# pingcap-incubator/tinysql

Hardware: AMD Instinct MI355X
Metric: probed rows/sec on int64-key inner hash join (higher is better)
Workload: dtype int64; 1 GPU; SELECT count(*) FROM probe JOIN build ON k: 1e+08 x 1e+08 int64-key inner hash join per GPU, J-uniq-shuffled, hit ratio 1.0, build side resident in HBM; build key range 27 bits <= 28: packed route (2-byte entries against direct-address images) — keys beyond 28 bits (31 if unique) take the 64-bit route, see general_keys_64bit_route; probe_rows_per_gpu=100000000, build_rows_per_gpu=100000000, parallelism=single GPU

## Files before the change

### __graft_entry__.py

```python
import os
import subprocess
import sys

ROOT = os.path.dirname(os.path.abspath(__file__))
if ROOT not in sys.path:
    sys.path.insert(0, ROOT)


PIPELINED = {"tsq_join.resusage": (("k_lds_probe_count", "k_da_partition2p"), 3), "tsq_unionscan.resusage": (("k_us_",), 9),
             "tsq_lookup.resusage": (("k_lk_", "k_rg_"), 6),
             "tsq_insert.resusage": (("k_ins_", "k_aid_"), 7),
             "tsq_dupcheck.resusage": (("k_dc_", "k_rows_equal"), 17),
             "tsq_mvcc.resusage": (("k_mv_",), 12),
             "tsq_mvcc_write.resusage": (("k_mw_",), 8)}


def check_no_spills():
    import re

    total = 0
    for fname, (kernels, at_least) in PIPELINED.items():
        text = open(os.path.join(ROOT, "tinysql_amd", "csrc", fname)).read()
        seen = 0
        for m in re.finditer(r"Function Name: (\S+).*?ScratchSize \[bytes/lane\]: (\d+)", text, re.S):
            if any(k in m.group(1) for k in kernels):
                seen += 1
                if int(m.group(2)) != 0:
                    raise RuntimeError("%s spills %s bytes/lane: these kernels must not use scratch" % (m.group(1), m.group(2)))
        if seen < at_least:
            raise RuntimeError("resource-usage remarks of the kernels of %s not found (%d)" % (fname, seen))
        total += seen
    return total


def check_partition_fit():
    import re

    text = open(os.path.join(ROOT, "tinysql_amd", "csrc", "tsq_join.resusage")).read()
    seen = 0
    for m in re.finditer(r"Function Name: (\S*k_da_partition2pILi(\d+)E\S*).*?VGPRs: (\d+).*?LDS Size \[bytes/block\]: (\d+)", text, re.S):
        name, nt, vgprs, lds = m.group(1), int(m.group(2)), int(m.group(3)), int(m.group(4))
        seen += 1
        if vgprs > 128:
            raise RuntimeError("%s uses %d VGPRs: more than 128 leave fewer than 4 waves per SIMD" % (name, vgprs))
        if lds * (2 if nt == 512 else 1) > 160 * 1024:
            raise RuntimeError("%s uses %d bytes of LDS per workgroup: %d workgroup(s) per CU do not fit 160 KB" % (name, lds, 2 if nt == 512 else 1))
    if seen < 3:
        raise RuntimeError("resource-usage remarks of k_da_partition2p not found (%d)" % seen)
    return seen


def build():
    env = dict(os.environ)
    env.setdefault("HIPCC", "/opt/rocm/bin/hipcc")
    subprocess.run(["make", "-C", os.path.join(ROOT, "tinysql_amd", "csrc"), "-j4", "ARCH=gfx950"], check=True, env=env)
    check_no_spills()
    check_partition_fit()
    subprocess.run(["make", "-C", os.path.join(ROOT, "tinysql_amd", "host")], check=True)
    subprocess.run(["make", "-C", os.path.join(ROOT, "oracle")], check=True)
    subprocess.run(["make", "-C", os.path.join(ROOT, "tests", "hostsim")], check=True)
    import tinysql_amd
    from tinysql_amd import _lib
    _lib.load()


def smoke():
    import numpy as np

    from oracle import binding as orc
    from tests import gpu_helpers as G
    from tests import helpers as H
    from tinysql_amd import _abi as abi
    from tinysql_amd import _lib
    from tinysql_amd import expression as E
    from tinysql_amd.chunk import Chunk, Column

    rng = np.random.default_rng(1)
    n = 20000
    t = [abi.I64, abi.I64]
    left = Chunk([Column(abi.I64, rng.integers(0, 3000, n), rng.random(n) > 0.05), Column(abi.I64, rng.integers(-99, 99, n))])
    right = Chunk([Column(abi.I64, rng.integers(0, 3000, n), rng.random(n) > 0.05), Column(abi.I64, rng.integers(-99, 99, n))])
    with _lib.Context(0) as ctx:
        keep = []
        conds = [E.ScalarFunction("gt", E.ScalarFunction("plus", E.Column(1, abi.I64), E.Column(3, abi.I64)), E.Constant(0))]
        cfg = H.join_cfg(t, t, [0], [0], abi.JOIN_LEFT_OUTER, 1, conds, (), keep)
        want = orc.hash_join(cfg, right, left)
        got = G.run_join(ctx, cfg, right, left)
        assert H.rows_equal_unordered(got, want), "smoke: join rows differ from the oracle"
        c, s, x = G.run_join(ctx, cfg, right, left, count_only=True, checksum=True)
        assert c == want.NumRows() and (s, x) == orc.rows_checksum(want), "smoke: join checksum differs"
        aggs = [(abi.AGG_FIRSTROW, 0, abi.I64), (abi.AGG_SUM, 1, abi.I64), (abi.AGG_COUNT, -1, abi.I64)]
        acfg = H.agg_cfg(t, [0], aggs)
        assert H.rows_equal_unordered(G.run_agg(ctx, acfg, left, [abi.I64] * 3), orc.hash_agg(acfg, left, 4, 4)), "smoke: agg differs"
        from tinysql_amd.chunk import StrColumn
        words = [None if i % 7 == 0 else ("k%03d" % (i % 40)).encode() * (1 + i % 3) for i in range(n)]
        schk = Chunk([StrColumn(words), left.columns[1]])
        se = E.ScalarFunction("and", E.ScalarFunction("le", E.ScalarFunction("ifnull", E.Column(0, abi.BYTES), E.Constant("k020")), E.Constant("k020k020")),
                              E.ScalarFunction("gt", E.ScalarFunction("plus", E.ScalarFunction("length", E.Column(0, abi.BYTES)), E.Column(1, abi.I64)), E.Constant(0)))
        ce = E.CompiledExpr(ctx, [se])
        try:
            assert ce.VecEval(schk).values() == orc.expr_eval(E.compile_expr(se), schk)[0].values(), "smoke: string expression differs"
        finally:
            ce.close()
        from tinysql_amd import distsql
        raw = orc.encode_rows(left)
        dec, used = distsql.decode_rows(ctx, raw, left.types(), n)
        assert used == raw.size and dec.rows() == orc.decode_rows(raw, left.types(), n)[1].rows(), "smoke: row decode differs"
        assert G.run_sort(ctx, left, [0, 1], [False, True]).rows() == orc.sort_rows(left, [0, 1], [False, True]).rows(), "smoke: sort differs"
        from tinysql_amd import rowcodec as RC
        vals, offs = orc.rowcodec_encode(left, [1, 2])
        scan = RC.NewChunkDecoder(ctx, [RC.ColInfo(2, RC.TypeLonglong), RC.ColInfo(1, RC.TypeLonglong)]).DecodeToChunk(vals, offs)
        assert scan.rows() == orc.rowcodec_decode(vals, offs, None, [(2, abi.I64), (1, abi.I64)])[1].rows(), "smoke: stored-row decode differs"
        from tinysql_amd import tablecodec
        hs = rng.integers(-(1 << 62), 1 << 62, 1000)
        keys = tablecodec.EncodeRowKeysWithHandles(ctx, 41, hs)
        assert bytes(keys[:19]) == orc.encode_row_key(41, int(hs[0])) and (tablecodec.DecodeRowKeys(ctx, keys) == hs).all(), "smoke: record keys differ"
        resp_chunk = Chunk([left.columns[0], StrColumn(words), left.columns[1]])
        raw2, offs2 = distsql.encode_rows(ctx, resp_chunk)
        assert bytes(raw2) == bytes(orc.encode_rows(resp_chunk)), "smoke: response bytes with a string column differ"
        back = distsql.decode_chunks(ctx, distsql.response_chunks(raw2, offs2), resp_chunk.types())
        assert back.rows() == resp_chunk.rows(), "smoke: chunked response decode differs"
        from tinysql_amd import chunk_codec, coprocessor
        from tinysql_amd.gpu_pipeline import drain_device
        wire = chunk_codec.Codec(ctx, resp_chunk.types()).Encode(resp_chunk)
        assert wire == orc.WireChunk.from_chunk(resp_chunk).encode(), "smoke: wire chunk bytes differ"
        assert chunk_codec.Codec(ctx, resp_chunk.types()).Decode(wire)[0].to_chunk().rows() == resp_chunk.rows(), "smoke: wire chunk decode differs"
        ikeys, ioffs = orc.encode_index_keys(resp_chunk, 41, 2, hs[:resp_chunk.NumRows()], np.ones(resp_chunk.NumRows(), np.uint8))
        itypes = resp_chunk.types() + [abi.I64]
        iscan = coprocessor.indexScanExec(ctx, itypes, 3, coprocessor.indexScanExec.PrimaryKeyIsSigned, ikeys, ioffs)
        got_rows = [r for ch in drain_device(iscan) for r in ch.rows()]
        assert got_rows == orc.decode_index_kv(ikeys.tobytes(), ioffs, None, None, 3, itypes, 1)[1].rows(), "smoke: index scan differs"
        wchunk = Chunk([left.columns[0], StrColumn(words), left.columns[1]])
        wvals, woffs = tablecodec.EncodeRow(ctx, wchunk, [1, 2, 300])
        ovals, ooffs = orc.rowcodec_encode(wchunk, [1, 2, 300])
        assert bytes(wvals) == bytes(ovals) and (woffs == ooffs).all(), "smoke: stored-row encode differs"
        whs = np.arange(n, dtype=np.int64) - 7
        gk, gko, gv, gvo, gd = tablecodec.GenIndexKeys(ctx, 41, 3, True, Chunk(wchunk.columns[:2]), whs)
        in_key = np.array([None in r for r in Chunk(wchunk.columns[:2]).rows()])
        ok, oko = orc.encode_index_keys(Chunk(wchunk.columns[:2]), 41, 3, whs, in_key.astype(np.uint8))
        assert bytes(gk) == bytes(ok) and (gko == oko).all() and (gd == ~in_key).all() and gvo[-1] == 8 * int((~in_key).sum()) + int(in_key.sum()), "smoke: index entries differ"
        kb = Chunk([left.columns[0], StrColumn([None if i % 13 == 0 else b"w%d" % (i % 50) for i in range(n)]), left.columns[1]])
        kp = Chunk([right.columns[0], StrColumn([None if i % 11 == 0 else b"w%d" % (i % 60) for i in range(n)]), right.columns[1]])
        kcfg = H.join_cfg(kp.types(), kb.types(), [0, 1], [0, 1], abi.JOIN_LEFT_OUTER, 1)
        kstats = []
        kgot = G.run_join(ctx, kcfg, kb, kp, chunk_rows=1 << 20, radix=abi.RADIX_FORCE, stats_out=kstats)
        assert kstats[0].probe_route == abi.ROUTE_KEYREC and H.rows_equal_unordered(kgot, orc.hash_join(kcfg, kb, kp)), "smoke: key-record join differs"
        kconds = [E.ScalarFunction("gt", E.ScalarFunction("plus", E.Column(2, abi.I64), E.Column(5, abi.I64)), E.Constant(0))]
        ccfg = H.join_cfg(kp.types(), kb.types(), [0, 1], [0, 1], abi.JOIN_LEFT_OUTER, 1, kconds, (), keep)
        cstats = []
        cgot = G.run_join(ctx, ccfg, kb, kp, chunk_rows=1 << 20, radix=abi.RADIX_FORCE, stats_out=cstats)
        assert cstats[0].probe_route == abi.ROUTE_KEYREC and H.rows_equal_unordered(cgot, orc.hash_join(ccfg, kb, kp)), "smoke: key-record join with a condition differs"
        saggs = [(abi.AGG_FIRSTROW, 1, abi.BYTES), (abi.AGG_SUM, 2, abi.I64), (abi.AGG_COUNT, -1, abi.I64)]
        scfg = H.agg_cfg(kb.types(), [1], saggs)
        sstats = []
        sgot = G.run_agg(ctx, scfg, kb, [abi.BYTES, abi.I64, abi.I64], chunk_rows=1 << 20, fast=abi.AGGFAST_FORCE, stats_out=sstats)
        assert sstats[0].build_partitioned == 3 and H.rows_equal_unordered(sgot, orc.hash_agg(scfg, kb, 4, 4)), "smoke: dictionary aggregate differs"
        ordered = orc.sort_rows(left, [0], [False])
        st_got = G.run_agg(ctx, acfg, ordered, [abi.I64] * 3, stream=True)
        assert H.rows_equal_unordered(st_got, orc.hash_agg(acfg, left, 4, 4)), "smoke: stream aggregate differs"
        from tinysql_amd import executor as X
        from tinysql_amd.gpu_pipeline import DeviceChunk, DeviceTableScan, GpuUnionScanExec
        uh = np.arange(2000, dtype=np.int64) * 2
        ua = uh[::5] + 1
        dirty = X.DirtyTable()
        for h_ in ua:
            dirty.AddRow(h_)
        for h_ in uh[::7]:
            dirty.DeleteRow(h_)
        table = DeviceChunk.from_host(ctx, Chunk([Column(abi.I64, uh), Column(abi.I64, uh * 3)]))
        try:
            us = GpuUnionScanExec(ctx, DeviceTableScan(ctx, table, 512), dirty, Chunk([Column(abi.I64, ua), Column(abi.I64, ua * 3)]), [], 0, False)
            us_rows = [r for ch in drain_device(us) for r in ch.rows()]
        finally:
            table.free()
        us_want = np.sort(np.concatenate([np.setdiff1d(uh, uh[::7]), ua]))
        assert us_rows == [(int(v), int(v) * 3) for v in us_want], "smoke: union scan differs"
        from tinysql_amd.gpu_pipeline import GpuIndexLookUpExecutor
        lh = np.sort(rng.choice(np.arange(-9000, 9000), 3000, replace=False)).astype(np.int64)
        lv, lw = rng.integers(0, 500, 3000), rng.integers(-99, 99, 3000)
        lvals, loffs = tablecodec.EncodeRow(ctx, Chunk([Column(abi.I64, lv), Column(abi.I64, lw)]), [1, 2])
        ltable = coprocessor.DeviceTable(ctx, tablecodec.EncodeRowKeysWithHandles(ctx, 41, lh), lvals, loffs)
        try:
            ih = np.concatenate([lh, 20000 + np.arange(200)])
            iv = np.concatenate([lv, rng.integers(0, 500, 200)])
            io = np.lexsort((ih, iv))
            ik, iko, ivl, ivo, _ = tablecodec.GenIndexKeys(ctx, 41, 5, False, Chunk([Column(abi.I64, iv[io])]), ih[io])
            linfo = [RC.ColInfo(1, RC.TypeLonglong), RC.ColInfo(2, RC.TypeLonglong), RC.ColInfo(-1, RC.TypeLonglong, IsPKHandle=True)]
            for keep_order in (True, False):
                iscan2 = coprocessor.indexScanExec(ctx, [abi.I64, abi.I64], 1, coprocessor.indexScanExec.PrimaryKeyIsSigned, ik, iko, ivl, ivo)
                lk = GpuIndexLookUpExecutor(ctx, iscan2, ltable, linfo, [], keep_order, 64, 1024)
                lrows = [r for ch in drain_device(lk) for r in ch.rows()]
                lwant = []
                at, batch = 0, 64
                while at < ih.size:
                    th = ih[io][at:at + batch]
                    th = th[np.isin(th, lh)]
                    lwant += (th if keep_order else np.sort(th)).tolist()
                    at, batch = at + batch, min(2 * batch, 1024)
                pos = np.searchsorted(lh, np.array(lwant, dtype=np.int64))
                assert lrows == [(int(lv[p]), int(lw[p]), int(lh[p])) for p in pos], "smoke: index lookup differs (keep_order=%s)" % keep_order
        finally:
# ... 73 lines not shown
```

### tinysql_amd/csrc/tsq_join.hip

```cpp
#include "tsq_stage.h"
#include "tsq_jointable.h"
#include "tsq_buildpart.h"
#include "tsq_ldsprobe.h"
#include "tsq_keyrec.h"
#include "tsq_dajoin.h"
#include "tsq_damat.h"
#include "tsq_damat_dup.h"

#include <chrono>
#include <deque>
#include <memory>

struct KeySpec {
    int32_t n_keys;
    int32_t bidx[TSQ_MAX_KEYS];
    int32_t pidx[TSQ_MAX_KEYS];
    int32_t skip_high;
};

template <bool MULTI>
__device__ __forceinline__ bool load_kw(const tsq_colset& cs, const int32_t* idx, int n_keys, bool skip_high,
                                        int64_t row, uint64_t& kw) {
    if (!MULTI) {
        const int c = idx[0];
// ... 912 lines not shown
                    if (r->pending) { TSQ_TRY(settle_batch(j, r.get())); break; }
        } else {
            TSQ_HIP(&j->hdr, hipStreamSynchronize(ctx->stream));
            rb->copy_on = nullptr;
            rb->free_device();
            rb->on_host = true;
        }
    } else {
        TSQ_HIP(&j->hdr, hipStreamSynchronize(ctx->stream));
        for (auto& b : rb->notnull) b.release();
    }
    j->total_out += out_rows;
    j->st.out_rows += out_rows;
    j->results.push_back(std::move(rb));
    return TSQ_OK;
}

bool radix_eligible(const tsq_join* j, int64_t nrows, const uint8_t* selected_dev) {
    if (j->radix_mode == TSQ_RADIX_OFF) return false;
    if (!j->count_only || j->checksum || j->multi || j->general_cfg || j->never_match || j->chained) return false;
    if (nrows <= 0 || nrows > 0x7fffffffLL) return false;
    if (j->radix_mode == TSQ_RADIX_FORCE) return true;
    return j->nbuckets * 64 >= ((uint64_t)12 << 20) && nrows >= (4 << 20);
}

bool da_multi_ok(const tsq_join* j);
bool da_multi_count_eligible(const tsq_join* j, int64_t nrows, const uint8_t* selected_dev) {
    if (j->radix_mode == TSQ_RADIX_OFF || j->packing_mode == TSQ_RADIX_OFF || !j->multi || !da_multi_ok(j) || j->da_state < 0) return false;
    if (!j->count_only || j->checksum || j->general_cfg || j->never_match || j->chained) return false;
    if (nrows <= 0 || nrows > 0x7fffffffLL) return false;
    if (j->radix_mode == TSQ_RADIX_FORCE || j->packing_mode == TSQ_RADIX_FORCE) return true;
    return nrows >= (4 << 20);
}

struct RadixPlan {
    bool lds;
    uint32_t bits, S, nf;
};
RadixPlan radix_plan_for(const tsq_join* j) {
    RadixPlan pl{false, TSQ_RADIX_MIN_BITS, 1, 1};
    const int64_t nf_env = tsq_knob(j->ctx, TSQ_KNOB_LDS_NF_MAX, 0), pb_env = tsq_knob(j->ctx, TSQ_KNOB_RADIX_PB_MAX, 0);
    const bool want_lds = tsq_knob(j->ctx, TSQ_KNOB_RADIX_KERNEL_L2, 0) == 0;
    if (want_lds && j->tb >= TSQ_RADIX_MIN_BITS && (uint64_t)j->bs * 64 <= TSQ_LDS_IMAGE_MAX) {
        uint32_t nf_max = (uint32_t)(TSQ_LDS_IMAGE_MAX / ((uint64_t)j->bs * 64));
        if (nf_env >= 1 && (uint32_t)nf_env < nf_max) nf_max = (uint32_t)nf_env;
        uint32_t k = 0;
        while ((2u << k) <= nf_max) k++;
        int pb = (int)j->tb - (int)k;
        if (pb < TSQ_RADIX_MIN_BITS) pb = TSQ_RADIX_MIN_BITS;
        if (pb > TSQ_RADIX_MAX_BITS) pb = TSQ_RADIX_MAX_BITS;
        if (pb_env >= TSQ_RADIX_MIN_BITS && pb_env < pb) pb = (int)pb_env;
        const uint32_t fpp = 1u << (j->tb - (uint32_t)pb);
        pl.lds = true;
        pl.bits = (uint32_t)pb;
        pl.nf = fpp < nf_max ? fpp : nf_max;
        pl.S = (fpp + pl.nf - 1) / pl.nf;
        return pl;
    }
    const double slice_target = 1.5 * 1024 * 1024;
    const double parts = (double)j->nbuckets * 64.0 / slice_target;
    uint32_t bits = TSQ_RADIX_MIN_BITS;
    while (bits < 10 && (double)(1u << bits) < parts) bits++;
    if (j->tb && bits > j->tb) bits = j->tb;
    pl.bits = bits;
    return pl;
}

tsq_status batch_begin(tsq_join* j, DevEvent*& re, bool ev2 = false) {
    re = nullptr;
    if (ev2) TSQ_HIP(&j->hdr, hipEventRecord(j->ev[2], j->ctx->stream));
    const int64_t every = tsq_knob(j->ctx, TSQ_KNOB_JOIN_BATCH_TIMING, 4), b = j->st.radix_batches;
    if (every <= 0 || b % every != every - 1) return TSQ_OK;
    DevEvent* slot = j->rev[b % tsq_join::RING];
    for (int e = 0; e < 3; e++)
        TSQ_HIP(&j->hdr, slot[e].create());
    j->rev_batch1[b % tsq_join::RING] = b + 1;
    TSQ_HIP(&j->hdr, hipEventRecord(slot[0], j->ctx->stream));
    re = slot;
    return TSQ_OK;
}
tsq_status batch_mark(tsq_join* j, DevEvent* re, int e) {
    if (re) TSQ_HIP(&j->hdr, hipEventRecord(re[e], j->ctx->stream));
    return TSQ_OK;
}
tsq_status batch_end(tsq_join* j, DevEvent* re) {
    if (!re) return TSQ_OK;
    TSQ_HIP(&j->hdr, hipEventRecord(re[2], j->ctx->stream));
    j->probe_ev_slot = (int)(re - j->rev[0]) / 3;
    j->have_probe_ev = true;
    return TSQ_OK;
}
tsq_status radix_probe(tsq_join* j, const tsq_colset& pcs, int64_t nrows) {
    tsq_ctx* ctx = j->ctx;
    tsq_handle_hdr* h = &j->hdr;
    RadixStore st;
    memset(&st, 0, sizeof st);
    const RadixPlan pl = radix_plan_for(j);
    st.bits = pl.bits;
    st.R = 8;
    const uint32_t P = 1u << st.bits;
    constexpr int NT = 1024, K = 16, T = NT * K;
    const double lam = (double)nrows / ((double)P * 8.0);
    st.cap = (uint32_t)(lam * 1.08 + 8.0 * sqrt(lam) + 2.0 * T / 64.0 + 64.0);
    st.cap = (st.cap + 15u) & ~15u;
    const size_t nregions = (size_t)P * 8;
    if (nregions * st.cap >= 0xffffffffULL) return tsq_fail(h, TSQ_ERR_UNSUPPORTED, "radix probe batch too large");
    const size_t ctl_words32 = nregions + 16;
    const size_t ctl_bytes = ((ctl_words32 * 4 + 511) & ~(size_t)511) + 8 * TSQ_RADIX_QSTRIDE * 8;
    TSQ_TRY(j->rkeys.reserve(ctx, h, nregions * st.cap * 8 + 256));
    TSQ_TRY(j->rctl.reserve(ctx, h, ctl_bytes));
    TSQ_TRY(j->rvend.reserve(ctx, h, nregions * 4));
    TSQ_TRY(j->rovf.reserve(ctx, h, (size_t)nrows * 8 + 64));
    st.keys = j->rkeys.as<uint64_t>();
    st.cursor = j->rctl.as<uint32_t>();
    st.ovf_count = st.cursor + nregions;
    st.queue = (unsigned long long*)((char*)j->rctl.p + ((ctl_words32 * 4 + 511) & ~(size_t)511));
    st.valid_end = j->rvend.as<uint32_t>();
    st.ovf_keys = j->rovf.as<uint64_t>();
    st.ovf_cap = (uint32_t)nrows;
    j->da_ctl_dirty();
    TSQ_HIP(h, hipMemsetAsync(j->rctl.p, 0, ctl_bytes, ctx->stream));
    TSQ_HIP(h, hipMemsetAsync(j->rvend.p, 0xff, nregions * 4, ctx->stream));

    RadixSrc src;
    memset(&src, 0, sizeof src);
    const int kc = j->ks.pidx[0];
    src.data = pcs.data[kc];
    src.nulls = pcs.nulls[kc];
    src.type = pcs.type[kc];
    src.skip_high = j->ks.skip_high;
    src.nrows = nrows;
    const int64_t ntiles = (nrows + T - 1) / T;
    const int pgrid = (int)std::min<int64_t>(ntiles, ctx->num_cus);
    DevEvent* re;
    TSQ_TRY(batch_begin(j, re));
    hipLaunchKernelGGL((k_radix_partition<NT, K, 4, 0, false, true>), dim3(pgrid), dim3(NT), 0, ctx->stream, src, st);
    TSQ_HIP(h, hipGetLastError());
    TSQ_TRY(batch_mark(j, re, 1));
    RadixProbeArgs pa;
    memset(&pa, 0, sizeof pa);
    pa.st = st;
    fill_table(j, pa.t);
    pa.counters = j->counters.as<unsigned long long>();
    if (pl.lds) {
        constexpr int LNT = 1024;
        LdsProbeArgs la;
        memset(&la, 0, sizeof la);
        la.st = st;
        la.t = pa.t;
        la.S = pl.S;
        la.nf = pl.nf;
        la.unique = j->unique ? 1u : 0u;
        la.counters = pa.counters;
        const size_t lds = (size_t)pl.nf * j->bs * 64 + (size_t)(LNT / 64) * TSQ_LDS_RING_BYTES;
        const int lgrid = std::max(1, ctx->num_cus / 8) * 8;
        if (tsq_knob(ctx, TSQ_KNOB_LDS_PROF, 0) != 0) {
            DevBuf pb;
            TSQ_TRY(pb.reserve(ctx, h, 64));
            la.prof = pb.as<unsigned long long>();
            TSQ_HIP(h, hipMemsetAsync(pb.p, 0, 64, ctx->stream));
            TSQ_HIP(h, hipFuncSetAttribute((const void*)k_lds_probe_count<LNT, true>, hipFuncAttributeMaxDynamicSharedMemorySize, (int)lds));
            hipLaunchKernelGGL((k_lds_probe_count<LNT, true>), dim3(lgrid), dim3(LNT), lds, ctx->stream, la);
            unsigned long long pf[8];
            TSQ_HIP(h, hipMemcpyAsync(ctx->pinned + 24, pb.p, 64, hipMemcpyDeviceToHost, ctx->stream));
            TSQ_HIP(h, hipStreamSynchronize(ctx->stream));
            memcpy(pf, ctx->pinned + 24, 64);
            pb.release();
            const double nw = (double)lgrid * (LNT / 64);
            fprintf(stderr, "[lds-prof] P=2^%u S=%u nf=%u bs=%u waves=%.0f | per wave kcycles: imageA %.1f loadwait %.1f step %.1f probe %.1f drainB %.1f total %.1f | probes/wave %.0f\n",
                    st.bits, pl.S, pl.nf, j->bs, nw, pf[0] / nw / 1e3, pf[1] / nw / 1e3, pf[2] / nw / 1e3, pf[3] / nw / 1e3, pf[4] / nw / 1e3, pf[5] / nw / 1e3, pf[6] / nw);
        } else {
            TSQ_HIP(h, hipFuncSetAttribute((const void*)k_lds_probe_count<LNT>, hipFuncAttributeMaxDynamicSharedMemorySize, (int)lds));
            hipLaunchKernelGGL((k_lds_probe_count<LNT>), dim3(lgrid), dim3(LNT), lds, ctx->stream, la);
        }
    } else {
        const int per_xcd = std::max(1, ctx->num_cus / 8) * 6;
        hipLaunchKernelGGL((k_radix_probe_count<2>), dim3(per_xcd * 8), dim3(256), 0, ctx->stream, pa);
    }
    TSQ_HIP(h, hipGetLastError());
    hipLaunchKernelGGL(k_radix_probe_ovf, dim3(ctx->num_cus), dim3(256), 0, ctx->stream, pa);
    TSQ_HIP(h, hipGetLastError());
    TSQ_TRY(batch_end(j, re));
    j->st.kernel_launches += 3;
    j->st.radix_batches++;
    j->st.radix_bits = (int32_t)st.bits;
    j->st.probe_route = pl.lds ? TSQ_ROUTE_RADIX_LDS : TSQ_ROUTE_RADIX_L2;
    return TSQ_OK;
}

struct DaGeom {
    uint32_t P, cap;
    size_t nregions, ent_bytes, ctl_bytes;
};
DaGeom da_geometry(uint32_t pbits, uint32_t ebits, int64_t nrows, int T) {
    DaGeom g;
    g.P = 1u << pbits;
    const double tiles = ceil((double)nrows / T);
    const double lam = std::max((double)nrows / ((double)g.P * 8.0), ceil(tiles / 8.0) * std::min<double>((double)T, (double)nrows) / (double)g.P);
    g.cap = (uint32_t)(lam * 1.08 + 8.0 * sqrt(lam) + 2.0 * T / 64.0 + 64.0);
    g.cap = (g.cap + 63u) & ~63u;
    g.nregions = (size_t)g.P * 8;
    g.ent_bytes = g.nregions * g.cap * (ebits > 16 ? 4 : 2) + 256;
    g.ctl_bytes = ((g.nregions + 16) * 4 + 511) & ~(size_t)511;
    return g;
}

template <class... P, class... A>
hipError_t da_launch(void (*fn)(P...), dim3 grid, dim3 block, size_t lds, hipStream_t stream, const A&... args) {
    if (lds) {
        const hipError_t e = hipFuncSetAttribute((const void*)fn, hipFuncAttributeMaxDynamicSharedMemorySize, (int)lds);
        if (e != hipSuccess) return e;
    }
    hipLaunchKernelGGL(fn, grid, block, lds, stream, args...);
    return hipGetLastError();
}
struct DaBuildTimer {
    tsq_join* j;
    DevEvent e0, e1;
    explicit DaBuildTimer(tsq_join* j_) : j(j_) {}
    hipError_t start() {
        hipError_t e = e0.create();
        if (e == hipSuccess) e = e1.create();
        return e == hipSuccess ? hipEventRecord(e0, j->ctx->stream) : e;
    }
    hipError_t stop() { return hipEventRecord(e1, j->ctx->stream); }
    ~DaBuildTimer() {
        float ms = 0;
        if (e0 && e1 && hipEventElapsedTime(&ms, e0, e1) == hipSuccess) j->da_build_ms += ms;
    }
};
DaStore da_store(const tsq_join* j, const DaGeom& g, int64_t rows, void* ent, void* ctl, void* vend, void* ovf) {
    DaStore st;
    memset(&st, 0, sizeof st);
    st.ent = ent;
    st.cursor = (uint32_t*)ctl;
    st.ovf_count = st.cursor + g.nregions;
    st.valid_end = (uint32_t*)vend;
    st.ovf = (uint32_t*)ovf;
    st.ovf_cap = (uint32_t)rows;
    st.bits = j->da_pbits;
    st.ebits = j->da_ebits;
    st.cap = g.cap;
    return st;
}
hipError_t da_clear(tsq_ctx* ctx, void* ctl, void* vend, const DaGeom& g) {
    const hipError_t e = hipMemsetAsync(ctl, 0, g.ctl_bytes, ctx->stream);
    return e == hipSuccess ? hipMemsetAsync(vend, 0xff, g.nregions * 4, ctx->stream) : e;
}
struct DaBuildStore {
    DevBuf ent, idx, ctl, vend, ovf, ovfi, nnm, pay[TSQ_DA_MAXCOLS];
    tsq_status reserve(tsq_join* j, const DaGeom& g, int64_t nb, bool ids, int ncols = -1, bool nulls = false) {
        tsq_ctx* ctx = j->ctx;
        tsq_handle_hdr* h = &j->hdr;
        const size_t slots = g.nregions * g.cap;
        tsq_status s = ent.reserve(ctx, h, g.ent_bytes);
        if (s == TSQ_OK && ids) s = idx.reserve(ctx, h, slots * 4 + 256);
        if (s == TSQ_OK) s = ctl.reserve(ctx, h, g.ctl_bytes);
        if (s == TSQ_OK) s = vend.reserve(ctx, h, g.nregions * 4);
        if (s == TSQ_OK) s = ovf.reserve(ctx, h, (size_t)nb * 4 + 64);
        if (s == TSQ_OK && (ids || ncols >= 0)) s = ovfi.reserve(ctx, h, (size_t)nb * 4 + 64);
        for (int v = 0; v < ncols && s == TSQ_OK; v++) s = pay[v].reserve(ctx, h, slots * 8 + 256);
        if (s == TSQ_OK && nulls) s = nnm.reserve(ctx, h, slots + 256);
        return s;
    }
    DaStore store(const tsq_join* j, const DaGeom& g, int64_t nb) const {
        DaStore st = da_store(j, g, nb, ent.p, ctl.p, vend.p, ovf.p);
        st.idx = idx.as<uint32_t>();
        st.ovf_idx = ovfi.as<uint32_t>();
        return st;
    }
    DaColStore col_store(const tsq_join* j, const DaGeom& g, int64_t nb, int ncols, bool nulls) const {
        DaColStore cs;
        memset(&cs, 0, sizeof cs);
        cs.st = store(j, g, nb);
        cs.st.miss_count = cs.st.ovf_count + 1;
        for (int v = 0; v < ncols; v++) cs.pay[v] = pay[v].as<uint64_t>();
        cs.nnmask = nulls ? nnm.as<uint8_t>() : nullptr;
        return cs;
    }
    hipError_t clear(tsq_ctx* ctx, const DaGeom& g) { return da_clear(ctx, ctl.p, vend.p, g); }
};
enum DaIds { DA_IDS_NONE, DA_IDS_LISTS, DA_IDS_ALL };
tsq_status da_probe_store(tsq_join* j, const DaGeom& g, int64_t nrows, DaIds ids, bool miss, DaStore& st) {
    tsq_ctx* ctx = j->ctx;
    tsq_handle_hdr* h = &j->hdr;
    TSQ_TRY(j->rkeys.reserve(ctx, h, g.ent_bytes));
    if (ids == DA_IDS_ALL) TSQ_TRY(j->ridx.reserve(ctx, h, g.nregions * g.cap * 4 + 256));
    TSQ_TRY(j->rctl.reserve(ctx, h, g.ctl_bytes));
    TSQ_TRY(j->rvend.reserve(ctx, h, g.nregions * 4));
    TSQ_TRY(j->rovf.reserve(ctx, h, (size_t)nrows * 4 + 64));
    if (ids != DA_IDS_NONE) TSQ_TRY(j->rovfidx.reserve(ctx, h, (size_t)nrows * 4 + 64));
    if (miss) TSQ_TRY(j->rmiss.reserve(ctx, h, (size_t)nrows * 4 + 64));
    st = da_store(j, g, nrows, j->rkeys.p, j->rctl.p, j->rvend.p, j->rovf.p);
    if (ids == DA_IDS_ALL) st.idx = j->ridx.as<uint32_t>();
    if (ids != DA_IDS_NONE) {
        st.ovf_idx = j->rovfidx.as<uint32_t>();
        st.miss_count = st.ovf_count + 1;
        st.miss = j->rmiss.as<uint32_t>();
    }
    return TSQ_OK;
}
tsq_status da_clear_batch(tsq_join* j, const DaGeom& g) {
    tsq_ctx* ctx = j->ctx;
    tsq_handle_hdr* h = &j->hdr;
    const size_t n_pc = (size_t)g.P + 1;
    TSQ_TRY(j->tkcnt.reserve(ctx, h, n_pc * 8 + 64));
    j->da_ctl_dirty();
    TSQ_HIP(h, da_clear(ctx, j->rctl.p, j->rvend.p, g));
    TSQ_HIP(h, hipMemsetAsync(j->tkcnt.p, 0, n_pc * 8, ctx->stream));
    TSQ_HIP(h, hipMemsetAsync(ctx->dscratch + 52, 0, 16, ctx->stream));
    return TSQ_OK;
}
struct DaSizes {
    int64_t part_rows, ovf_rows, miss_rows;
};
tsq_status da_queue_sizes(tsq_join* j, const DaStore& st, const unsigned long long* total, const void* ovf, size_t ovf_bytes) {
    tsq_ctx* ctx = j->ctx;
    tsq_handle_hdr* h = &j->hdr;
    ctx->pinned[53] = 0;
    TSQ_HIP(h, hipMemcpyAsync(ctx->pinned + 52, total, 8, hipMemcpyDeviceToHost, ctx->stream));
    TSQ_HIP(h, hipMemcpyAsync(ctx->pinned + 53, ovf, ovf_bytes, hipMemcpyDeviceToHost, ctx->stream));
    TSQ_HIP(h, hipMemcpyAsync(ctx->pinned + 54, st.miss_count, 4, hipMemcpyDeviceToHost, ctx->stream));
    return TSQ_OK;
}
tsq_status da_wait_sizes(tsq_join* j, bool outer, DaSizes& z) {
    tsq_ctx* ctx = j->ctx;
// ... 3532 lines not shown
```

### tinysql_amd/csrc/tsq_ldsprobe.h

```cpp
#ifndef TSQ_LDSPROBE_H
#define TSQ_LDSPROBE_H

#include "tsq_radix.h"

#define TSQ_LDS_IMAGE_MAX (128 * 1024)
#define TSQ_LDS_RING 128
#define TSQ_LDS_RING_BYTES (TSQ_LDS_RING * 10)
#define TSQ_LDS_RING_BYTES_EMIT (TSQ_LDS_RING * 14)
#define TSQ_LDS_MAXPAY 2

typedef unsigned long long tsq_u64x2 __attribute__((ext_vector_type(2)));
__device__ __forceinline__ ulonglong2 nt_load16(const void* p) {
    const tsq_u64x2 v = __builtin_nontemporal_load(reinterpret_cast<const tsq_u64x2*>(p));
    return make_ulonglong2(v.x, v.y);
}

__device__ __forceinline__ void async_nt_load16(tsq_u64x2& dst, const void* p) {
#ifdef TSQ_LDS_KEYS_NT
    asm volatile("global_load_dwordx4 %0, %1, off nt" : "=v"(dst) : "v"(p) : "memory");
#else
    asm volatile("global_load_dwordx4 %0, %1, off" : "=v"(dst) : "v"(p) : "memory");
#endif
}
template <int YOUNGER>
__device__ __forceinline__ void async_wait(tsq_u64x2& dst) {
    asm volatile("s_waitcnt vmcnt(%1)" : "+v"(dst) : "n"(YOUNGER) : "memory");
}

struct LdsProbeArgs {
    RadixStore st;
    JoinTable t;
    uint32_t S;
    uint32_t nf;
    uint32_t unique;
    unsigned long long* counters;
    unsigned long long* prof;
    unsigned long long* tk_cnt;
    uint64_t* out_probe[1 + TSQ_LDS_MAXPAY];
    uint64_t* out_build[1 + TSQ_LDS_MAXPAY];
    int32_t probe_src[1 + TSQ_LDS_MAXPAY], build_src[1 + TSQ_LDS_MAXPAY];
    int32_t n_out_probe, n_out_build;
    const uint64_t* bpay[TSQ_LDS_MAXPAY];
    const uint64_t* bcol[TSQ_LDS_MAXPAY];
    unsigned long long* ovf_cursor;
};

template <int NT, bool PROF = false, int MODE = 0>
__global__ void __launch_bounds__(NT) k_lds_probe_count(LdsProbeArgs a) {
    constexpr int NW = NT / 64;
    unsigned long long pf[8] = {0, 0, 0, 0, 0, 0, 0, 0};
    auto now = [&]() -> unsigned long long { return PROF ? (unsigned long long)__builtin_readcyclecounter() : 0ull; };
    const unsigned long long t_begin = now();
    constexpr int IMG_R = TSQ_LDS_IMAGE_MAX / 16 / NT;
    constexpr int PRE_R = MODE == 2 ? IMG_R - 2 : IMG_R;
    constexpr int D = 4;
    static_assert(NW % 8 == 0, "NW / 8 waves per XCC region");
    extern __shared__ __align__(16) unsigned char s_dyn[];
    __shared__ uint32_t s_len[8];
    __shared__ uint32_t s_tk[2];
    __shared__ uint32_t s_next;
    __shared__ unsigned long long s_total;
    const uint32_t tid = threadIdx.x, lane = tid & 63u;
    const uint32_t wave = (uint32_t)__builtin_amdgcn_readfirstlane(tid >> 6);
    const uint32_t vx = blockIdx.x & 7u;
    const uint32_t P = 1u << a.st.bits, NP = P >> 3;
    const uint32_t tb = a.t.tb, bs = a.t.bs, sh = 64u - tb;
    const uint32_t fpp = 1u << (tb - a.st.bits);
    const uint32_t ntk = NP * a.S;
    const uint32_t img_words = a.nf * bs * TSQ_BUCKET;
    uint64_t* s_img = reinterpret_cast<uint64_t*>(s_dyn);
    uint64_t* s_ring = s_img + img_words + (size_t)wave * TSQ_LDS_RING;
    uint16_t* s_hop = reinterpret_cast<uint16_t*>(s_img + img_words + (size_t)NW * TSQ_LDS_RING) + (size_t)wave * TSQ_LDS_RING;
    uint32_t* s_gix = reinterpret_cast<uint32_t*>(reinterpret_cast<unsigned char*>(s_img + img_words) + (size_t)NW * TSQ_LDS_RING * 10) + (size_t)wave * TSQ_LDS_RING;
    __shared__ unsigned long long s_tkcnt;
    __shared__ uint32_t s_out;
    auto take = [&]() -> uint32_t {
        return (uint32_t)__hip_atomic_fetch_add(&a.st.queue[vx * TSQ_RADIX_QSTRIDE], 1ull, __ATOMIC_RELAXED, __HIP_MEMORY_SCOPE_AGENT);
    };
    uint32_t pend = 0;
    if (tid == 0) {
        s_total = 0;
        s_tk[0] = take();
        s_tk[1] = take();
        pend = take();
    }
    __syncthreads();
    auto first_slice = [&](uint32_t tk, uint32_t& nfi) -> uint32_t {
        const uint32_t pi = tk / a.S, sub = tk - pi * a.S;
        const uint32_t rest = fpp - sub * a.nf;
        nfi = rest < a.nf ? rest : a.nf;
        return (pi * 8u + vx) * fpp + sub * a.nf;
    };
    ulonglong2 pre[PRE_R];
    auto image_load = [&](uint32_t tk) {
        uint32_t nfi;
        const uint32_t f0 = first_slice(tk < ntk ? tk : 0u, nfi);
        const uint32_t n16 = nfi * bs * (TSQ_BUCKET / 2);
        const ulonglong2* src = reinterpret_cast<const ulonglong2*>(a.t.keys + (size_t)f0 * bs * TSQ_BUCKET);
#pragma unroll
        for (int j = 0; j < PRE_R; j++) {
            const uint32_t i = (uint32_t)j * NT + tid;
            pre[j] = nt_load16(src + (i < n16 ? i : 0u));
        }
    };
    uint32_t tk = (uint32_t)__builtin_amdgcn_readfirstlane(s_tk[0]);
    image_load(tk);
    uint32_t cnt = 0;
    for (uint32_t it = 0; tk < ntk; it++) {
        const unsigned long long t0 = now();
        uint32_t nfi;
        const uint32_t f0 = first_slice(tk, nfi);
        const uint32_t p = (tk / a.S) * 8u + vx;
        {
            const uint32_t n16 = nfi * bs * (TSQ_BUCKET / 2);
            ulonglong2* dst = reinterpret_cast<ulonglong2*>(s_img);
            ulonglong2 late[IMG_R - PRE_R + 1];
            const ulonglong2* src = reinterpret_cast<const ulonglong2*>(a.t.keys + (size_t)f0 * bs * TSQ_BUCKET);
#pragma unroll
            for (int j = PRE_R; j < IMG_R; j++) {
                const uint32_t i = (uint32_t)j * NT + tid;
                late[j - PRE_R] = nt_load16(src + (i < n16 ? i : 0u));
            }
#pragma unroll
            for (int j = 0; j < PRE_R; j++) {
                const uint32_t i = (uint32_t)j * NT + tid;
                if (i < n16) dst[i] = pre[j];
            }
#pragma unroll
            for (int j = PRE_R; j < IMG_R; j++) {
                const uint32_t i = (uint32_t)j * NT + tid;
                if (i < n16) dst[i] = late[j - PRE_R];
            }
        }
        if (tid < 8) s_len[tid] = radix_region_len(a.st, P, p, tid);
        if (tid == 9) s_next = 0;
        if (MODE == 1 && tid == 8) s_tkcnt = 0;
        if (MODE == 2 && tid == 8) {
            s_tkcnt = a.tk_cnt[(size_t)vx * ntk + tk];
            s_out = 0;
        }
        const uint32_t cnt0 = cnt;
        __syncthreads();
        if (PROF) pf[0] += now() - t0;
        const uint32_t tkn = (uint32_t)__builtin_amdgcn_readfirstlane(s_tk[(it + 1) & 1u]);
        uint32_t maxlen = 0;
#pragma unroll
        for (int r = 0; r < 8; r++) {
            const uint32_t l = (uint32_t)__builtin_amdgcn_readfirstlane(s_len[r]);
            maxlen = l > maxlen ? l : maxlen;
        }
        const uint32_t spr = (maxlen + 511u) / 512u, nsc = spr * 8u;
        const uint64_t* pbase = a.st.keys + (size_t)p * 8u * a.st.cap;
        const uint32_t pgbase = (uint32_t)((size_t)p * 8u * a.st.cap);
        struct Sc {
            uint32_t rbase, rlen, off0;
        };
        auto locate = [&](uint32_t id) -> Sc {
            uint32_t r = 0;
#pragma unroll
            for (uint32_t q = 1; q < 8; q++) r += id >= q * spr ? 1u : 0u;
            Sc x;
            x.rlen = (uint32_t)__builtin_amdgcn_readfirstlane(s_len[r]);
            x.rbase = r * a.st.cap;
            x.off0 = (id - r * spr) * 512u;
            return x;
        };
        auto chunk_load = [&](const Sc& sc, uint32_t d, tsq_u64x2& v, uint32_t& nv, uint32_t& gi) {
            const uint32_t off = sc.off0 + d * 128u + lane * 2u;
            nv = off + 1u < sc.rlen ? 2u : (off < sc.rlen ? 1u : 0u);
            gi = pgbase + sc.rbase + off;
            async_nt_load16(v, pbase + (sc.rbase + (off < sc.rlen ? off : 0u)));
        };
        auto draw = [&]() -> uint32_t {
            uint32_t g = 0;
            if (lane == 0) g = atomicAdd(&s_next, 1u);
            return g;
        };
        uint32_t cur = (uint32_t)__builtin_amdgcn_readfirstlane(draw());
        uint32_t nxt = (uint32_t)__builtin_amdgcn_readfirstlane(draw());
        uint32_t gpend = draw();
        Sc sc_cur = locate(cur), sc_nxt = locate(nxt);
        tsq_u64x2 v[D];
        uint32_t nv[D], gi[D];
#pragma unroll
        for (int d = 0; d < D; d++) chunk_load(sc_cur, (uint32_t)d, v[d], nv[d], gi[d]);
        image_load(tkn);
        uint32_t qh = 0, qt = 0;
        auto push = [&](bool on, uint64_t w, uint32_t hop, uint32_t gx) {
            const uint64_t m = __ballot(on);
            if (m) {
                if (on) {
                    const uint32_t pos = (qt + __builtin_amdgcn_mbcnt_hi((uint32_t)(m >> 32), __builtin_amdgcn_mbcnt_lo((uint32_t)m, 0u))) & (TSQ_LDS_RING - 1);
                    s_ring[pos] = w;
                    s_hop[pos] = (uint16_t)hop;
                    if (MODE == 2) s_gix[pos] = gx;
                }
                qt += (uint32_t)__popcll(m);
                __builtin_amdgcn_fence(__ATOMIC_RELEASE, "wavefront");
            }
        };
        auto probe_round = [&](uint32_t n) {
            const unsigned long long tp = now();
            __builtin_amdgcn_fence(__ATOMIC_ACQUIRE, "wavefront");
            const uint32_t pos = (qh + lane) & (TSQ_LDS_RING - 1);
            qh += n;
            bool go_on = false;
            uint64_t x = 0, gbkt = 0;
            uint32_t hop = 0, gx = 0, mm = 0;
            uint64_t ppay[TSQ_LDS_MAXPAY] = {0, 0};
            if (lane < n) {
                x = s_ring[pos];
                hop = s_hop[pos];
                if (MODE == 2) {
                    gx = s_gix[pos];
#pragma unroll
                    for (int vv = 0; vv < TSQ_LDS_MAXPAY; vv++)
                        if (a.st.pay[vv]) ppay[vv] = a.st.pay[vv][gx];
                }
                if (x == TSQ_EMPTY_KEY) {
                    cnt += a.t.sent_count;
                    if (MODE == 2 && a.t.sent_count) {
                        const uint64_t key = tsq_unmix64(x);
                        const uint64_t row0 = s_tkcnt + atomicAdd(&s_out, a.t.sent_count);
                        for (uint32_t i = 0; i < a.t.sent_count; i++) {
                            const uint32_t brow = a.t.sent_rows[i];
                            for (int oc = 0; oc < a.n_out_probe; oc++) a.out_probe[oc][row0 + i] = a.probe_src[oc] < 0 ? key : ppay[a.probe_src[oc]];
                            for (int oc = 0; oc < a.n_out_build; oc++) a.out_build[oc][row0 + i] = a.build_src[oc] < 0 ? key : a.bcol[a.build_src[oc]][brow];
                        }
                    }
                } else {
                    const uint32_t xh = (uint32_t)(x >> 32), xl = (uint32_t)x;
                    uint32_t lb = __umulhi(__builtin_amdgcn_alignbit(xh, xl, 32u - tb), bs) + hop;
                    lb = lb >= bs ? lb - bs : lb;
                    const uint32_t lbkt = __umul24((xh >> (sh - 32u)) - f0, bs) + lb;
                    const uint64_t* bk = s_img + (size_t)lbkt * TSQ_BUCKET;
                    const ulonglong2* b = reinterpret_cast<const ulonglong2*>(bk);
                    const ulonglong2 q0 = b[lane & 3u], q1 = b[(lane + 1u) & 3u], q2 = b[(lane + 2u) & 3u], q3 = b[(lane + 3u) & 3u];
                    const uint64_t last = bk[TSQ_BUCKET - 1];
                    const uint32_t c = (uint32_t)(q0.x == x) + (uint32_t)(q0.y == x) + (uint32_t)(q1.x == x) + (uint32_t)(q1.y == x) +
                                       (uint32_t)(q2.x == x) + (uint32_t)(q2.y == x) + (uint32_t)(q3.x == x) + (uint32_t)(q3.y == x);
                    cnt += c;
                    go_on = last != TSQ_EMPTY_KEY && !(a.unique && c) && hop + 1u < bs;
                    if (MODE == 2 && c) {
                        mm = (uint32_t)(q0.x == x) | ((uint32_t)(q0.y == x) << 1) | ((uint32_t)(q1.x == x) << 2) | ((uint32_t)(q1.y == x) << 3) |
                             ((uint32_t)(q2.x == x) << 4) | ((uint32_t)(q2.y == x) << 5) | ((uint32_t)(q3.x == x) << 6) | ((uint32_t)(q3.y == x) << 7);
                        gbkt = (uint64_t)f0 * bs + lbkt;
                    }
                }
            }
            if (MODE == 2) {
                const uint64_t any = __ballot(mm != 0);
                if (any) {
                    const uint32_t c = (uint32_t)__popc(mm);
                    uint32_t tot;
                    const uint32_t pre = wave_excl_scan_u32(c, &tot);
                    uint32_t base = 0;
                    if (lane == 0) base = atomicAdd(&s_out, tot);
                    base = (uint32_t)__builtin_amdgcn_readfirstlane(base);
                    const uint64_t key = tsq_unmix64(x);
                    uint64_t row = s_tkcnt + base + pre;
                    while (mm) {
                        const uint32_t i = (uint32_t)__builtin_ctz(mm);
                        mm &= mm - 1u;
                        const uint32_t slot = 2u * ((lane + (i >> 1)) & 3u) + (i & 1u);
                        for (int oc = 0; oc < a.n_out_probe; oc++) a.out_probe[oc][row] = a.probe_src[oc] < 0 ? key : ppay[a.probe_src[oc]];
                        for (int oc = 0; oc < a.n_out_build; oc++)
                            a.out_build[oc][row] = a.build_src[oc] < 0 ? key : a.bpay[a.build_src[oc]][gbkt * TSQ_BUCKET + slot];
                        row++;
                    }
                }
            }
            push(go_on, x, hop + 1u, gx);
            if (PROF) {
                pf[3] += now() - tp;
                pf[6]++;
            }
        };
        auto step = [&](uint64_t w, bool valid, uint32_t gx) {
            push(valid && (((uint32_t)(w >> 32) >> (sh - 32u)) - f0) < nfi, w, 0u, gx);
            while (qt - qh >= 64u) probe_round(64u);
        };
        while (cur < nsc) {
#pragma unroll
            for (int d = 0; d < D; d++) {
                const unsigned long long tw = now();
                async_wait<D - 1>(v[d]);
                const unsigned long long ts = now();
                step(v[d].x, nv[d] >= 1, gi[d]);
                step(v[d].y, nv[d] >= 2, gi[d] + 1u);
                if (PROF) {
                    pf[1] += ts - tw;
                    pf[2] += now() - ts;
                }
                chunk_load(sc_nxt, (uint32_t)d, v[d], nv[d], gi[d]);
            }
            cur = nxt;
            sc_cur = sc_nxt;
            nxt = (uint32_t)__builtin_amdgcn_readfirstlane(gpend);
            gpend = draw();
            sc_nxt = locate(nxt);
        }
        const unsigned long long td = now();
        asm volatile("s_waitcnt vmcnt(0)" : "+v"(v[0]), "+v"(v[1]), "+v"(v[2]), "+v"(v[3]) : : "memory");
        static_assert(D == 4, "drain lists v[0..3]");
        while (qt != qh) probe_round(qt - qh < 64u ? qt - qh : 64u);
        if (MODE == 1) {
            const uint64_t wsum = wave_sum_u64((uint64_t)(cnt - cnt0));
            if (lane == 0 && wsum) atomicAdd(&s_tkcnt, (unsigned long long)wsum);
        }
        __syncthreads();
        if (MODE == 1 && tid == 8) a.tk_cnt[(size_t)vx * ntk + tk] = s_tkcnt;
        if (PROF) pf[4] += now() - td;
        if (tid == 0) {
            s_tk[it & 1u] = pend;
            pend = take();
        }
        tk = tkn;
    }
    if (PROF && lane == 0) {
        pf[5] = now() - t_begin;
        pf[2] -= pf[3];
#pragma unroll
        for (int i = 0; i < 8; i++) atomicAdd(&a.prof[i], pf[i]);
    }
    const uint64_t ws = wave_sum_u64(cnt);
    if (lane == 0 && ws) atomicAdd(&s_total, (unsigned long long)ws);
    __syncthreads();
    if (MODE == 0 && tid == 0 && s_total) atomicAdd(&a.counters[0], s_total);
}

static __global__ void __launch_bounds__(256) k_lds_emit_ovf(LdsProbeArgs a) {
    uint32_t n = *a.st.ovf_count;
    n = n < a.st.ovf_cap ? n : a.st.ovf_cap;
    for (uint32_t i = blockIdx.x * 256 + threadIdx.x; i < n; i += gridDim.x * 256) {
        const uint64_t w = a.st.ovf_keys[i], key = tsq_unmix64(w);
        uint64_t ppay[TSQ_LDS_MAXPAY] = {0, 0};
#pragma unroll
        for (int vv = 0; vv < TSQ_LDS_MAXPAY; vv++)
            if (a.st.ovf_pay[vv]) ppay[vv] = a.st.ovf_pay[vv][i];
        auto emit = [&](uint64_t bval_idx, bool by_row) {
            const unsigned long long row = atomicAdd(a.ovf_cursor, 1ull);
            for (int oc = 0; oc < a.n_out_probe; oc++) a.out_probe[oc][row] = a.probe_src[oc] < 0 ? key : ppay[a.probe_src[oc]];
            for (int oc = 0; oc < a.n_out_build; oc++)
                a.out_build[oc][row] = a.build_src[oc] < 0 ? key : (by_row ? a.bcol[a.build_src[oc]][bval_idx] : a.bpay[a.build_src[oc]][bval_idx]);
        };
        if (w == TSQ_EMPTY_KEY) {
            for (uint32_t q = 0; q < a.t.sent_count; q++) emit(a.t.sent_rows[q], true);
        } else {
            for_each_slot_w(a.t, w, [&](uint64_t slot) { emit(slot, false); });
        }
    }
}

static __global__ void __launch_bounds__(256) k_table_payload(const uint64_t* keys, const uint32_t* vals, const uint64_t* col, uint64_t* out, uint64_t nslots) {
    for (uint64_t i = (uint64_t)blockIdx.x * 256 + threadIdx.x; i < nslots; i += (uint64_t)gridDim.x * 256)
        out[i] = keys[i] != TSQ_EMPTY_KEY ? col[vals[i]] : 0ull;
}

#endif
```

Baseline: 853.4 billion rows/s.

## Specialize count-only LDS probe with continuation buffer and uniqueness template

Adds a count-mode (MODE 0) specialization of the LDS probe kernel. Fresh keys are batched two at a time into a ring of plain 8-byte entries. Keys that must hop to the next bucket go to a small per-wave continuation buffer that is consumed first in the next round, so the ring no longer stores hop or global-index side data. A compile-time UNIQ flag replaces per-match counting with a ballot of hits, and the host picks the instantiation from the table's uniqueness. This shrinks ring LDS and per-round bookkeeping, at the cost of more template variants and more intricate ring/continuation ordering logic that could be wrong.

Result: no change. 848.8 billion rows/s (median of 2 runs) (-0.5%).

```diff
diff --git a/__graft_entry__.py b/__graft_entry__.py
--- a/__graft_entry__.py
+++ b/__graft_entry__.py
@@ -47,6 +47,24 @@
             raise RuntimeError("%s uses %d bytes of LDS per workgroup: %d workgroup(s) per CU do not fit 160 KB" % (name, lds, 2 if nt == 512 else 1))
     if seen < 3:
         raise RuntimeError("resource-usage remarks of k_da_partition2p not found (%d)" % seen)
+    ring = {0: 128 * 8 + 64 * 10, 1: 128 * 10, 2: 128 * 14}
+    probes, parts = set(), 0
+    for unit in ("tsq_join.resusage", "tsq_agg.resusage"):
+        text = open(os.path.join(ROOT, "tinysql_amd", "csrc", unit)).read()
+        for m in re.finditer(r"Function Name: (\S*(k_lds_probe_count|k_radix_partition)ILi(\d+)E(?:Lb[01]ELi(\d)E)?\S*).*?ScratchSize \[bytes/lane\]: (\d+)"
+                             r".*?LDS Size \[bytes/block\]: (\d+)", text, re.S):
+            name, kind, nt, mode, scratch, lds = m.group(1), m.group(2), int(m.group(3)), m.group(4), int(m.group(5)), int(m.group(6))
+            if kind == "k_lds_probe_count":
+                probes.add(int(mode))
+                if scratch:
+                    raise RuntimeError("%s uses %d bytes of scratch per lane" % (name, scratch))
+                lds += 128 * 1024 + nt // 64 * ring[int(mode)]
+            else:
+                parts += 1
+            if lds > 160 * 1024:
+                raise RuntimeError("%s needs %d bytes of LDS per workgroup: more than 160 KB" % (name, lds))
+    if probes != {0, 1, 2} or parts < 7:
+        raise RuntimeError("resource-usage remarks of k_lds_probe_count / k_radix_partition not found (modes %s, %d partition kernels)" % (sorted(probes), parts))
     return seen
 
 
diff --git a/tinysql_amd/csrc/tsq_join.hip b/tinysql_amd/csrc/tsq_join.hip
--- a/tinysql_amd/csrc/tsq_join.hip
+++ b/tinysql_amd/csrc/tsq_join.hip
@@ -1088,15 +1088,18 @@
         la.nf = pl.nf;
         la.unique = j->unique ? 1u : 0u;
         la.counters = pa.counters;
-        const size_t lds = (size_t)pl.nf * j->bs * 64 + (size_t)(LNT / 64) * TSQ_LDS_RING_BYTES;
+        const size_t lds = (size_t)pl.nf * j->bs * 64 + (size_t)(LNT / 64) * TSQ_LDS_RING_BYTES_COUNT;
         const int lgrid = std::max(1, ctx->num_cus / 8) * 8;
-        if (tsq_knob(ctx, TSQ_KNOB_LDS_PROF, 0) != 0) {
+        const bool prof = tsq_knob(ctx, TSQ_KNOB_LDS_PROF, 0) != 0;
+        void (*const kern)(LdsProbeArgs) = prof ? (j->unique ? k_lds_probe_count<LNT, true, 0, true> : k_lds_probe_count<LNT, true, 0, false>)
+                                                : (j->unique ? k_lds_probe_count<LNT, false, 0, true> : k_lds_probe_count<LNT, false, 0, false>);
+        TSQ_HIP(h, hipFuncSetAttribute((const void*)kern, hipFuncAttributeMaxDynamicSharedMemorySize, (int)lds));
+        if (prof) {
             DevBuf pb;
             TSQ_TRY(pb.reserve(ctx, h, 64));
             la.prof = pb.as<unsigned long long>();
             TSQ_HIP(h, hipMemsetAsync(pb.p, 0, 64, ctx->stream));
-            TSQ_HIP(h, hipFuncSetAttribute((const void*)k_lds_probe_count<LNT, true>, hipFuncAttributeMaxDynamicSharedMemorySize, (int)lds));
-            hipLaunchKernelGGL((k_lds_probe_count<LNT, true>), dim3(lgrid), dim3(LNT), lds, ctx->stream, la);
+            hipLaunchKernelGGL(kern, dim3(lgrid), dim3(LNT), lds, ctx->stream, la);
             unsigned long long pf[8];
             TSQ_HIP(h, hipMemcpyAsync(ctx->pinned + 24, pb.p, 64, hipMemcpyDeviceToHost, ctx->stream));
             TSQ_HIP(h, hipStreamSynchronize(ctx->stream));
@@ -1106,8 +1109,7 @@
             fprintf(stderr, "[lds-prof] P=2^%u S=%u nf=%u bs=%u waves=%.0f | per wave kcycles: imageA %.1f loadwait %.1f step %.1f probe %.1f drainB %.1f total %.1f | probes/wave %.0f\n",
                     st.bits, pl.S, pl.nf, j->bs, nw, pf[0] / nw / 1e3, pf[1] / nw / 1e3, pf[2] / nw / 1e3, pf[3] / nw / 1e3, pf[4] / nw / 1e3, pf[5] / nw / 1e3, pf[6] / nw);
         } else {
-            TSQ_HIP(h, hipFuncSetAttribute((const void*)k_lds_probe_count<LNT>, hipFuncAttributeMaxDynamicSharedMemorySize, (int)lds));
-            hipLaunchKernelGGL((k_lds_probe_count<LNT>), dim3(lgrid), dim3(LNT), lds, ctx->stream, la);
+            hipLaunchKernelGGL(kern, dim3(lgrid), dim3(LNT), lds, ctx->stream, la);
         }
     } else {
         const int per_xcd = std::max(1, ctx->num_cus / 8) * 6;
diff --git a/tinysql_amd/csrc/tsq_ldsprobe.h b/tinysql_amd/csrc/tsq_ldsprobe.h
--- a/tinysql_amd/csrc/tsq_ldsprobe.h
+++ b/tinysql_amd/csrc/tsq_ldsprobe.h
@@ -1,5 +1,7 @@
 #ifndef TSQ_LDSPROBE_H
 #define TSQ_LDSPROBE_H
+
+#include <type_traits>
 
 #include "tsq_radix.h"
 
@@ -7,6 +9,8 @@
 #define TSQ_LDS_RING 128
 #define TSQ_LDS_RING_BYTES (TSQ_LDS_RING * 10)
 #define TSQ_LDS_RING_BYTES_EMIT (TSQ_LDS_RING * 14)
+#define TSQ_LDS_CONT 64
+#define TSQ_LDS_RING_BYTES_COUNT (TSQ_LDS_RING * 8 + TSQ_LDS_CONT * 10)
 #define TSQ_LDS_MAXPAY 2
 
 typedef unsigned long long tsq_u64x2 __attribute__((ext_vector_type(2)));
@@ -45,8 +49,9 @@
     unsigned long long* ovf_cursor;
 };
 
-template <int NT, bool PROF = false, int MODE = 0>
+template <int NT, bool PROF = false, int MODE = 0, bool UNIQ = false>
 __global__ void __launch_bounds__(NT) k_lds_probe_count(LdsProbeArgs a) {
+    static_assert(MODE == 0 || !UNIQ, "MODE 1 / 2 read a.unique at run time");
     constexpr int NW = NT / 64;
     unsigned long long pf[8] = {0, 0, 0, 0, 0, 0, 0, 0};
     auto now = [&]() -> unsigned long long { return PROF ? (unsigned long long)__builtin_readcyclecounter() : 0ull; };
@@ -72,6 +77,8 @@
     uint64_t* s_ring = s_img + img_words + (size_t)wave * TSQ_LDS_RING;
     uint16_t* s_hop = reinterpret_cast<uint16_t*>(s_img + img_words + (size_t)NW * TSQ_LDS_RING) + (size_t)wave * TSQ_LDS_RING;
     uint32_t* s_gix = reinterpret_cast<uint32_t*>(reinterpret_cast<unsigned char*>(s_img + img_words) + (size_t)NW * TSQ_LDS_RING * 10) + (size_t)wave * TSQ_LDS_RING;
+    uint64_t* s_cw = s_img + img_words + (size_t)NW * TSQ_LDS_RING + (size_t)wave * TSQ_LDS_CONT;
+    uint16_t* s_ch = reinterpret_cast<uint16_t*>(s_img + img_words + (size_t)NW * (TSQ_LDS_RING + TSQ_LDS_CONT)) + (size_t)wave * TSQ_LDS_CONT;
     __shared__ unsigned long long s_tkcnt;
     __shared__ uint32_t s_out;
     auto take = [&]() -> uint32_t {
@@ -167,7 +174,12 @@
         };
         auto chunk_load = [&](const Sc& sc, uint32_t d, tsq_u64x2& v, uint32_t& nv, uint32_t& gi) {
             const uint32_t off = sc.off0 + d * 128u + lane * 2u;
-            nv = off + 1u < sc.rlen ? 2u : (off < sc.rlen ? 1u : 0u);
+            if constexpr (MODE == 0) {
+                const int32_t rem = (int32_t)(sc.rlen - off);
+                nv = (uint32_t)(rem < 0 ? 0 : (rem > 2 ? 2 : rem));
+            } else {
+                nv = off + 1u < sc.rlen ? 2u : (off < sc.rlen ? 1u : 0u);
+            }
             gi = pgbase + sc.rbase + off;
             async_nt_load16(v, pbase + (sc.rbase + (off < sc.rlen ? off : 0u)));
         };
@@ -280,14 +292,117 @@
             push(valid && (((uint32_t)(w >> 32) >> (sh - 32u)) - f0) < nfi, w, 0u, gx);
             while (qt - qh >= 64u) probe_round(64u);
         };
+        const uint32_t sl_lo = f0 << (sh - 32u), sl_span = nfi << (sh - 32u);
+        const bool has_sent = (uint32_t)(((uint32_t)(TSQ_EMPTY_KEY >> 32) >> (sh - 32u)) - f0) < nfi;
+        uint32_t nc = 0;
+        auto round0 = [&](auto full, uint32_t n) {
+            const unsigned long long tp = now();
+            __builtin_amdgcn_fence(__ATOMIC_ACQUIRE, "wavefront");
+            const uint32_t c0 = nc;
+            const uint32_t pos = (qh - c0 + lane) & (TSQ_LDS_RING - 1);
+            qh += n - c0;
+            nc = 0;
+            auto B = [](bool p) -> uint64_t { return __builtin_amdgcn_ballot_w64(p); };
+            uint64_t gom = 0;
+            uint64_t x = 0;
+            uint32_t hop = 0;
+            constexpr bool FULL = decltype(full)::value;
+            const uint64_t vm = FULL ? ~0ull : ~0ull >> (64u - n);
+            {
+                x = s_ring[pos];
+                if (c0) {
+                    if (lane < c0) {
+                        x = s_cw[lane];
+                        hop = s_ch[lane];
+                    }
+                }
+                if constexpr (!FULL) x = __builtin_amdgcn_inverse_ballot_w64(vm) ? x : (uint64_t)sl_lo << 32;
+                const uint32_t xh = (uint32_t)(x >> 32), xl = (uint32_t)x;
+                uint32_t lb = __umulhi(__builtin_amdgcn_alignbit(xh, xl, 32u - tb), bs) + hop;
+                lb = lb - bs < lb ? lb - bs : lb;
+                const uint32_t lbkt = __umul24((xh - sl_lo) >> (sh - 32u), bs) + lb;
+                const uint64_t* bk = s_img + (size_t)lbkt * TSQ_BUCKET;
+                const ulonglong2* b = reinterpret_cast<const ulonglong2*>(bk);
+                const ulonglong2 q0 = b[lane & 3u], q1 = b[(lane + 1u) & 3u], q2 = b[(lane + 2u) & 3u], q3 = b[(lane + 3u) & 3u];
+                const uint64_t last = bk[TSQ_BUCKET - 1];
+                uint64_t gm = B(last != TSQ_EMPTY_KEY) & B(hop < bs - 1u) & vm;
+                uint64_t hm = 0;
+                uint32_t c = 0;
+                if constexpr (UNIQ) {
+                    hm = B(q0.x == x) | B(q0.y == x) | B(q1.x == x) | B(q1.y == x) | B(q2.x == x) | B(q2.y == x) | B(q3.x == x) | B(q3.y == x);
+                    hm &= vm;
+                    gm &= ~hm;
+                } else {
+                    c = (uint32_t)(q0.x == x) + (uint32_t)(q0.y == x) + (uint32_t)(q1.x == x) + (uint32_t)(q1.y == x) +
+                        (uint32_t)(q2.x == x) + (uint32_t)(q2.y == x) + (uint32_t)(q3.x == x) + (uint32_t)(q3.y == x);
+                    if constexpr (!FULL) c = __builtin_amdgcn_inverse_ballot_w64(vm) ? c : 0u;
+                }
+                if (has_sent) {
+                    const uint64_t sm = B(x == TSQ_EMPTY_KEY) & vm;
+                    if (sm) {
+                        const bool is_sent = __builtin_amdgcn_inverse_ballot_w64(sm);
+                        cnt += is_sent ? a.t.sent_count : 0u;
+                        c = is_sent ? 0u : c;
+                        hm &= ~sm;
+                        gm &= ~sm;
+                    }
+                }
+                cnt += UNIQ ? (__builtin_amdgcn_inverse_ballot_w64(hm) ? 1u : 0u) : c;
+                gom = gm;
+            }
+            if (gom) {
+                if (__builtin_amdgcn_inverse_ballot_w64(gom)) {
+                    const uint32_t i = __builtin_amdgcn_mbcnt_hi((uint32_t)(gom >> 32), __builtin_amdgcn_mbcnt_lo((uint32_t)gom, 0u));
+                    s_cw[i] = x;
+                    s_ch[i] = (uint16_t)(hop + 1u);
+                }
+                nc = (uint32_t)__popcll(gom);
+                __builtin_amdgcn_fence(__ATOMIC_RELEASE, "wavefront");
+            }
+            if (PROF) {
+                pf[3] += now() - tp;
+                pf[6]++;
+            }
+        };
+        auto fresh = [&](bool on, uint64_t m, uint32_t before, uint64_t w) {
+            if (on) s_ring[__builtin_amdgcn_mbcnt_hi((uint32_t)(m >> 32), __builtin_amdgcn_mbcnt_lo((uint32_t)m, qt + before)) & (TSQ_LDS_RING - 1)] = w;
+        };
+        auto step2 = [&](uint64_t w0, uint64_t w1, uint32_t nvv) {
+            const uint64_t m0 = __builtin_amdgcn_ballot_w64(nvv >= 1u) & __builtin_amdgcn_ballot_w64((uint32_t)((uint32_t)(w0 >> 32) - sl_lo) < sl_span);
+            const uint64_t m1 = __builtin_amdgcn_ballot_w64(nvv >= 2u) & __builtin_amdgcn_ballot_w64((uint32_t)((uint32_t)(w1 >> 32) - sl_lo) < sl_span);
+            const bool on0 = __builtin_amdgcn_inverse_ballot_w64(m0), on1 = __builtin_amdgcn_inverse_ballot_w64(m1);
+            if (m0 | m1) {
+                const uint32_t n0 = (uint32_t)__popcll(m0), n1 = (uint32_t)__popcll(m1);
+                if (qt - qh + n0 + n1 <= (uint32_t)TSQ_LDS_RING) {
+                    fresh(on0, m0, 0u, w0);
+                    fresh(on1, m1, n0, w1);
+                    qt += n0 + n1;
+                    __builtin_amdgcn_fence(__ATOMIC_RELEASE, "wavefront");
+                    while (qt - qh + nc >= 64u) round0(std::true_type{}, 64u);
+                } else {
+                    fresh(on0, m0, 0u, w0);
+                    qt += n0;
+                    __builtin_amdgcn_fence(__ATOMIC_RELEASE, "wavefront");
+                    while (qt - qh + nc >= 64u) round0(std::true_type{}, 64u);
+                    fresh(on1, m1, 0u, w1);
+                    qt += n1;
+                    __builtin_amdgcn_fence(__ATOMIC_RELEASE, "wavefront");
+                    while (qt - qh + nc >= 64u) round0(std::true_type{}, 64u);
+                }
+            }
+        };
         while (cur < nsc) {
 #pragma unroll
             for (int d = 0; d < D; d++) {
                 const unsigned long long tw = now();
                 async_wait<D - 1>(v[d]);
                 const unsigned long long ts = now();
-                step(v[d].x, nv[d] >= 1, gi[d]);
-                step(v[d].y, nv[d] >= 2, gi[d] + 1u);
+                if constexpr (MODE == 0) {
+                    step2(v[d].x, v[d].y, nv[d]);
+                } else {
+                    step(v[d].x, nv[d] >= 1, gi[d]);
+                    step(v[d].y, nv[d] >= 2, gi[d] + 1u);
+                }
                 if (PROF) {
                     pf[1] += ts - tw;
                     pf[2] += now() - ts;
@@ -303,7 +418,11 @@
         const unsigned long long td = now();
         asm volatile("s_waitcnt vmcnt(0)" : "+v"(v[0]), "+v"(v[1]), "+v"(v[2]), "+v"(v[3]) : : "memory");
         static_assert(D == 4, "drain lists v[0..3]");
-        while (qt != qh) probe_round(qt - qh < 64u ? qt - qh : 64u);
+        if constexpr (MODE == 0) {
+            while (qt - qh + nc) round0(std::false_type{}, qt - qh + nc < 64u ? qt - qh + nc : 64u);
+        } else {
+            while (qt != qh) probe_round(qt - qh < 64u ? qt - qh : 64u);
+        }
         if (MODE == 1) {
             const uint64_t wsum = wave_sum_u64((uint64_t)(cnt - cnt0));
             if (lane == 0 && wsum) atomicAdd(&s_tkcnt, (unsigned long long)wsum);
```
